# hku-mars/Voxel-SLAM

Measured on AMD Instinct MI355X. Metric: BA iterations/sec (10-frame window, 100k pts/scan), higher is better.
Workload: dtype f64; 1 GPU; cfg2: W=10, 100000 pts/scan, 50000 voxels per GPU, nnz=500000; global_voxels=50000, parallelism=voxel-shard x1, ranks_seen=1, collectives_per_lm_step=0, allreduce_doubles=0, lm_steps_accepted=2028, lm_steps_rejected=0

## Files before the change

### voxel-slam_amd/csrc/vxba_solve4.hpp

```cpp
#pragma once

typedef double s4v2 __attribute__((ext_vector_type(2)));

constexpr int S4_WAVES = 4;
constexpr int S4_THREADS = 64 * S4_WAVES;
constexpr int S4_ROW = 6;
constexpr int S4_BLK = 64 * S4_ROW + 6;
constexpr int S4_GSLOT = 64 * S4_ROW;

template <int W>
struct S4 {
  static constexpr int N = 6 * W, M = N - 6, B = W - 1;
  static constexpr int TC = 0;
  static constexpr int G = TC + (B > 0 ? B : 1) * S4_BLK;
  static constexpr int BV = G + (B > 0 ? B : 1) * S4_GSLOT;
  static constexpr int ZV = BV + 64;
  static constexpr int XS = ZV + 64;
  static constexpr int DOUBLES = XS + 64;
};

__device__ __forceinline__ double s4_rcp(double d) {
  const double r = __builtin_amdgcn_rcp(d);
  const double e = fma(-d, r, 1.0);
  const double t = fma(e, e, e);
  const double q = fma(r, t, r);
  return fabs(d) > 1e-300 ? q : 0.0;
}

__device__ __forceinline__ void s4_ldl6(double (&D)[21], double (&inv)[6]) {
#pragma unroll
  for (int p = 0; p < 6; p++) {
    inv[p] = s4_rcp(D[p * (p + 1) / 2 + p]);
    double col[6];
#pragma unroll
    for (int q = p + 1; q < 6; q++) col[q] = D[q * (q + 1) / 2 + p];
#pragma unroll
    for (int q = p + 1; q < 6; q++) {
      const double l = col[q] * inv[p];
#pragma unroll
      for (int r = p + 1; r <= q; r++) D[q * (q + 1) / 2 + r] = fma(-l, col[r], D[q * (q + 1) / 2 + r]);
      D[q * (q + 1) / 2 + p] = l;
    }
  }
}

__device__ __forceinline__ void s4_load_row(const double* p, double (&a)[6]) {
  const s4v2* v = reinterpret_cast<const s4v2*>(p);
  const s4v2 t0 = v[0], t1 = v[1], t2 = v[2];
  a[0] = t0[0]; a[1] = t0[1]; a[2] = t1[0]; a[3] = t1[1]; a[4] = t2[0]; a[5] = t2[1];
}
__device__ __forceinline__ void s4_store_row(double* p, const double (&a)[6]) {
  s4v2* v = reinterpret_cast<s4v2*>(p);
  v[0] = (s4v2){a[0], a[1]};
  v[1] = (s4v2){a[2], a[3]};
  v[2] = (s4v2){a[4], a[5]};
}

template <int W>
__device__ __forceinline__ void s4_apply(const double* lds, int t, int b, int lane, double (&T)[6]) {
  using C = S4<W>;
  double g[6];
  s4_load_row(lds + C::G + t * S4_GSLOT + lane * S4_ROW, g);
  const double* lr = lds + C::TC + t * S4_BLK + (6 * b) * S4_ROW;
#pragma unroll
  for (int c = 0; c < 6; c++) {
    double l[6];
    s4_load_row(lr + c * S4_ROW, l);
#pragma unroll
    for (int p = 0; p < 6; p++) T[c] = fma(-g[p], l[p], T[c]);
  }
}

constexpr int li_rec_len(int W) { return 1 + 12 * W + 6 * W + 36 * W * W; }
constexpr int li_out_len(int W) { return 6 * W + 12 * W + 1; }
template <int W, bool DBG>
__device__ __forceinline__ int lm_solve_body4(LMState* st, int c, double* lds, const double* __restrict__ li_rec = nullptr, double* __restrict__ li_out = nullptr,
                                               unsigned li_seq = 0) {
  using C = S4<W>;
  LMCtl& ctl = st->ctl[c];
  const int loop_done = ctl.done;
  constexpr int n = C::N, M = C::M, B = C::B;
  const int tid = threadIdx.x, lane = tid & 63;
  const int wave = __builtin_amdgcn_readfirstlane(tid >> 6);
  dbg_stamp(DBG && wave == 0, 4000, 0);
  dbg_stamp(DBG && wave == 0, 4000, 1);
  const double u = li_rec ? li_rec[0] : ctl.u;
  const double* __restrict__ li_x = li_rec ? li_rec + 1 : nullptr;
  const double* __restrict__ li_e = li_rec ? li_rec + 1 + 12 * W : nullptr;
  const double* __restrict__ li_E = li_rec ? li_rec + 1 + 18 * W : nullptr;
  const bool row_ok = lane < M;
  const int gi_row = row_ok ? 6 + lane : 0;

  constexpr int NQ = (B + S4_WAVES - 1) / S4_WAVES;
  double a0[NQ > 0 ? NQ : 1][6];
#pragma unroll
  for (int q = 0; q < NQ; q++) {
    const int b = wave + S4_WAVES * q;
    const int bb = b < B ? b : 0;
#pragma unroll
    for (int cc = 0; cc < 6; cc++) {
      const int col = 6 + 6 * bb + cc;
      const double h = st->Hwork[(size_t)col * n + gi_row];
      const double add = (li_E && gi_row >= 6 + 6 * bb) ? li_E[(size_t)col * n + gi_row] : 0.0;
      a0[q][cc] = row_ok ? (((col == gi_row) ? h + u * h : h) + add) : 0.0;
    }
  }
  double hii = 0.0, gi = 0.0, rhs0 = 0.0;
  double xcur[12];
  if (wave == 0) {
    hii = st->Hwork[(size_t)gi_row * n + gi_row];
    gi = st->Jwork[gi_row];
    const int fl = lane < W ? lane : 0;
#pragma unroll
    for (int k = 0; k < 12; k++) xcur[k] = li_x ? li_x[12 * fl + k] : ctl.x[12 * fl + k];
  }
  if (wave == 1 % S4_WAVES) rhs0 = row_ok ? (li_e ? li_e[gi_row] : 0.0) - st->Jwork[gi_row] : 0.0;
  if (loop_done) return 1;
  if (wave < B) s4_store_row(lds + C::TC + wave * S4_BLK + lane * S4_ROW, a0[0]);
  dbg_stamp(DBG && wave == 0, 4000, 2);

  int ap0 = -1, ap1 = -1, ap2 = -1;
  for (int s = 0; s < B; s++) {
    const int owner = s & (S4_WAVES - 1);
    double Ld[21], inv[6], g[6];
    if (wave == owner) {
      const int sq = s >> 2;
      const int ap = sq == 0 ? ap0 : (sq == 1 ? ap1 : ap2);
      double* trow = lds + C::TC + s * S4_BLK + lane * S4_ROW;
      double a[6];
      dbg_stamp(DBG, 4010 + s, 0);
      s4_load_row(trow, a);
      for (int t = ap + 1; t < s; t++) s4_apply<W>(lds, t, s, lane, a);
      if (DBG) { asm volatile("" :: "v"(a[0]), "v"(a[5])); dbg_stamp(true, 4010 + s, 1); }
      s4_store_row(trow, a);
      __builtin_amdgcn_wave_barrier();
      {
        const double* dr = lds + C::TC + s * S4_BLK + (6 * s) * S4_ROW;
        const s4v2 r0 = *reinterpret_cast<const s4v2*>(dr);
        const s4v2 r1 = *reinterpret_cast<const s4v2*>(dr + 6);
        const s4v2 r2a = *reinterpret_cast<const s4v2*>(dr + 12), r2b = *reinterpret_cast<const s4v2*>(dr + 14);
        const s4v2 r3a = *reinterpret_cast<const s4v2*>(dr + 18), r3b = *reinterpret_cast<const s4v2*>(dr + 20);
        const s4v2 r4a = *reinterpret_cast<const s4v2*>(dr + 24), r4b = *reinterpret_cast<const s4v2*>(dr + 26), r4c = *reinterpret_cast<const s4v2*>(dr + 28);
        const s4v2 r5a = *reinterpret_cast<const s4v2*>(dr + 30), r5b = *reinterpret_cast<const s4v2*>(dr + 32), r5c = *reinterpret_cast<const s4v2*>(dr + 34);
        Ld[0] = r0[0];
        Ld[1] = r1[0]; Ld[2] = r1[1];
        Ld[3] = r2a[0]; Ld[4] = r2a[1]; Ld[5] = r2b[0];
        Ld[6] = r3a[0]; Ld[7] = r3a[1]; Ld[8] = r3b[0]; Ld[9] = r3b[1];
        Ld[10] = r4a[0]; Ld[11] = r4a[1]; Ld[12] = r4b[0]; Ld[13] = r4b[1]; Ld[14] = r4c[0];
        Ld[15] = r5a[0]; Ld[16] = r5a[1]; Ld[17] = r5b[0]; Ld[18] = r5b[1]; Ld[19] = r5c[0]; Ld[20] = r5c[1];
      }
      if (DBG) { asm volatile("" :: "v"(Ld[0]), "v"(Ld[20])); dbg_stamp(true, 4010 + s, 2); }
      s4_ldl6(Ld, inv);
      if (DBG) { asm volatile("" :: "v"(inv[5])); dbg_stamp(true, 4010 + s, 3); }
      double l[6];
#pragma unroll
      for (int p = 0; p < 6; p++) {
        double acc = a[p];
#pragma unroll
        for (int q = 0; q < p; q++) acc = fma(-g[q], Ld[p * (p + 1) / 2 + q], acc);
        g[p] = acc;
        l[p] = acc * inv[p];
      }
      s4_store_row(trow, l);
      s4_store_row(lds + C::G + s * S4_GSLOT + lane * S4_ROW, g);
      if (sq == 0) ap0 = s; else if (sq == 1) ap1 = s; else ap2 = s;
      dbg_stamp(DBG, 4010 + s, 4);
    }
    if (s == 0) {
#pragma unroll
      for (int q = 1; q < NQ; q++) {
        const int b = wave + S4_WAVES * q;
        if (b < B) s4_store_row(lds + C::TC + b * S4_BLK + lane * S4_ROW, a0[q]);
      }
      if (wave == 1 % S4_WAVES) lds[C::BV + lane] = rhs0;
    }
    if (s < 9) dbg_stamp(DBG, 4000 + wave, 6 + 2 * s);
    __syncthreads();
    if (s < 9) dbg_stamp(DBG, 4000 + wave, 7 + 2 * s);
    if (wave == owner) {
      double bb[6];
      s4_load_row(lds + C::BV + 6 * s, bb);
      double br = lds[C::BV + lane];
      double z[6];
#pragma unroll
      for (int p = 0; p < 6; p++) {
        double acc = bb[p];
#pragma unroll
        for (int q = 0; q < p; q++) acc = fma(-bb[q], Ld[p * (p + 1) / 2 + q], acc);
        bb[p] = acc;
        z[p] = acc * inv[p];
      }
#pragma unroll
      for (int p = 0; p < 6; p++) br = fma(-g[p], z[p], br);
      const int d = lane - 6 * s;
      double zsel = z[0];
#pragma unroll
      for (int p = 1; p < 6; p++) zsel = (d == p) ? z[p] : zsel;
      if (d >= 0 && d < 6) lds[C::ZV + lane] = zsel;
      else lds[C::BV + lane] = br;
    }
    const bool next_owner = (s + 1 < B) && wave == ((s + 1) & (S4_WAVES - 1));
    if (!next_owner) {
      int budget = 2;
#pragma unroll
      for (int q = 0; q < (B + S4_WAVES - 1) / S4_WAVES; q++) {
        const int b = wave + S4_WAVES * q;
        int ap = q == 0 ? ap0 : (q == 1 ? ap1 : ap2);
        const bool must = b == s + 2;
        if (b > s && b < B && ap < s && (must || budget > 0)) {
          double* trow = lds + C::TC + b * S4_BLK + lane * S4_ROW;
          double T[6];
          s4_load_row(trow, T);
          while (ap < s && (must || budget > 0)) {
            s4_apply<W>(lds, ap + 1, b, lane, T);
            ap++;
            budget--;
          }
          s4_store_row(trow, T);
          if (q == 0) ap0 = ap; else if (q == 1) ap1 = ap; else ap2 = ap;
        }
      }
    }
  }
  __syncthreads();
  dbg_stamp(DBG && wave == 0, 4000, 3);
  if (wave != 0) return 0;

  double x = row_ok ? lds[C::ZV + lane] : 0.0;
  if constexpr (B > 0) {
    const int jb = (row_ok ? lane : 0) / 6, jc = (row_ok ? lane : 0) % 6;
    const double* lcol = lds + C::TC + jb * S4_BLK + jc;
    double Lr[6], Ln[6];
#pragma unroll
    for (int k = 0; k < 6; k++) Lr[k] = lcol[(M - 1 - k) * S4_ROW];
    for (int rb = B - 1; rb >= 0; rb--) {
      if (rb > 0) {
#pragma unroll
        for (int k = 0; k < 6; k++) Ln[k] = lcol[(6 * rb - 1 - k) * S4_ROW];
      }
#pragma unroll
      for (int k = 0; k < 6; k++) {
        const int r = 6 * rb + 5 - k;
        const double xr = readlane_f64(x, r);
        x = (lane < r) ? fma(-Lr[k], xr, x) : x;
      }
#pragma unroll
      for (int k = 0; k < 6; k++) Lr[k] = Ln[k];
    }
  }
  dbg_stamp(DBG, 4000, 4);
  if (row_ok) st->dxi[6 + lane] = x;
  if (lane < 6) st->dxi[lane] = 0.0;
  double* xs = lds + C::XS;
  if (lane < 6) xs[lane] = 0.0;
  if (row_ok) xs[6 + lane] = x;
  __builtin_amdgcn_wave_barrier();
  if (lane < W) {
    double dl[6];
#pragma unroll
    for (int k = 0; k < 6; k++) dl[k] = xs[6 * lane + k];
    double xn[9];
    lm_right_multiply_exp(xcur, dl, xn);
#pragma unroll
    for (int k = 0; k < 9; k++) __hip_atomic_store(&ctl.xt[12 * lane + k], xn[k], __ATOMIC_RELAXED, __HIP_MEMORY_SCOPE_AGENT);
#pragma unroll
    for (int k = 0; k < 3; k++) __hip_atomic_store(&ctl.xt[12 * lane + 9 + k], xcur[9 + k] + dl[3 + k], __ATOMIC_RELAXED, __HIP_MEMORY_SCOPE_AGENT);
    if (li_out) {
#pragma unroll
      for (int k = 0; k < 9; k++) li_out[6 * W + 12 * lane + k] = xn[k];
#pragma unroll
      for (int k = 0; k < 3; k++) li_out[6 * W + 12 * lane + 9 + k] = xcur[9 + k] + dl[3 + k];
    }
  }
  if (li_out) {
    if (row_ok) li_out[6 + lane] = x;
    if (lane < 6) li_out[lane] = 0.0;
    asm volatile("s_waitcnt vmcnt(0)" ::: "memory");
    __builtin_amdgcn_wave_barrier();
    if (lane == 0) li_out[18 * W] = (double)li_seq;
  }
  double part = row_ok ? x * (u * hii * x - gi) : 0.0;
#pragma unroll
  for (int off = 32; off > 0; off >>= 1) part += __shfl_down(part, off);
  if (lane == 0) ctl.q1 = 0.5 * part;
  if (DBG) { asm volatile("s_waitcnt vmcnt(0)" ::: "memory"); dbg_stamp(true, 4000, 5); }
  return 0;
}
```

Before: 21430 iterations/s.

## Keep block-Cholesky critical chain on wave 0 with register-carried next panel

```diff
diff --git a/voxel-slam_amd/csrc/vxba_solve4.hpp b/voxel-slam_amd/csrc/vxba_solve4.hpp
--- a/voxel-slam_amd/csrc/vxba_solve4.hpp
+++ b/voxel-slam_amd/csrc/vxba_solve4.hpp
@@ -69,6 +69,104 @@
 #pragma unroll
     for (int p = 0; p < 6; p++) T[c] = fma(-g[p], l[p], T[c]);
   }
+}
+
+template <int W>
+__device__ __forceinline__ void s4_apply_g(const double* lds, const double (&g)[6], int t, int b, double (&T)[6]) {
+  using C = S4<W>;
+  const double* lr = lds + C::TC + t * S4_BLK + (6 * b) * S4_ROW;
+#pragma unroll
+  for (int c = 0; c < 6; c++) {
+    double l[6];
+    s4_load_row(lr + c * S4_ROW, l);
+#pragma unroll
+    for (int p = 0; p < 6; p++) T[c] = fma(-g[p], l[p], T[c]);
+  }
+}
+
+template <int W>
+__device__ __forceinline__ void s4_rhs_step(double* lds, int s, int lane, const double (&Ld)[21], const double (&inv)[6], const double (&g)[6]) {
+  using C = S4<W>;
+  double bb[6];
+  s4_load_row(lds + C::BV + 6 * s, bb);
+  double br = lds[C::BV + lane];
+  double z[6];
+#pragma unroll
+  for (int p = 0; p < 6; p++) {
+    double acc = bb[p];
+#pragma unroll
+    for (int q = 0; q < p; q++) acc = fma(-bb[q], Ld[p * (p + 1) / 2 + q], acc);
+    bb[p] = acc;
+    z[p] = acc * inv[p];
+  }
+#pragma unroll
+  for (int p = 0; p < 6; p++) br = fma(-g[p], z[p], br);
+  const int d = lane - 6 * s;
+  double zsel = z[0];
+#pragma unroll
+  for (int p = 1; p < 6; p++) zsel = (d == p) ? z[p] : zsel;
+  const bool own = d >= 0 && d < 6;
+  lds[(own ? C::ZV : C::BV) + lane] = own ? zsel : br;
+}
+
+__device__ __forceinline__ void s4_stamp(bool on, int row, int slot) {
+  if (on) g_dbg[row * DBG_SLOTS + slot] = __builtin_readcyclecounter();
+}
+
+template <int W, bool DBG, bool FIRST, bool LAST>
+__device__ __forceinline__ void s4_chain_step(double* lds, int s, int lane, double (&a)[6], double (&nx)[6], double (&Ld)[21], double (&inv)[6], double (&g)[6]) {
+  using C = S4<W>;
+  double* trow = lds + C::TC + s * S4_BLK + lane * S4_ROW;
+  s4_stamp(DBG, 4010 + s, 0);
+  s4_store_row(trow, a);
+  __builtin_amdgcn_wave_barrier();
+  double Dn[21], invn[6], gn[6], l[6];
+  {
+    const double* dr = lds + C::TC + s * S4_BLK + (6 * s) * S4_ROW;
+    const s4v2 r0 = *reinterpret_cast<const s4v2*>(dr);
+    const s4v2 r1 = *reinterpret_cast<const s4v2*>(dr + 6);
+    const s4v2 r2a = *reinterpret_cast<const s4v2*>(dr + 12), r2b = *reinterpret_cast<const s4v2*>(dr + 14);
+    const s4v2 r3a = *reinterpret_cast<const s4v2*>(dr + 18), r3b = *reinterpret_cast<const s4v2*>(dr + 20);
+    const s4v2 r4a = *reinterpret_cast<const s4v2*>(dr + 24), r4b = *reinterpret_cast<const s4v2*>(dr + 26), r4c = *reinterpret_cast<const s4v2*>(dr + 28);
+    const s4v2 r5a = *reinterpret_cast<const s4v2*>(dr + 30), r5b = *reinterpret_cast<const s4v2*>(dr + 32), r5c = *reinterpret_cast<const s4v2*>(dr + 34);
+    Dn[0] = r0[0];
+    Dn[1] = r1[0]; Dn[2] = r1[1];
+    Dn[3] = r2a[0]; Dn[4] = r2a[1]; Dn[5] = r2b[0];
+    Dn[6] = r3a[0]; Dn[7] = r3a[1]; Dn[8] = r3b[0]; Dn[9] = r3b[1];
+    Dn[10] = r4a[0]; Dn[11] = r4a[1]; Dn[12] = r4b[0]; Dn[13] = r4b[1]; Dn[14] = r4c[0];
+    Dn[15] = r5a[0]; Dn[16] = r5a[1]; Dn[17] = r5b[0]; Dn[18] = r5b[1]; Dn[19] = r5c[0]; Dn[20] = r5c[1];
+  }
+  if constexpr (!FIRST) {
+    s4_rhs_step<W>(lds, s - 1, lane, Ld, inv, g);
+    if constexpr (!LAST) {
+      s4_load_row(lds + C::TC + (s + 1) * S4_BLK + lane * S4_ROW, nx);
+      s4_apply_g<W>(lds, g, s - 1, s + 1, nx);
+    }
+  }
+  if (DBG) { if (!FIRST && !LAST) asm volatile("" :: "v"(nx[0]), "v"(nx[5])); s4_stamp(true, 4010 + s, 1); }
+  if (DBG) { asm volatile("" :: "v"(Dn[0]), "v"(Dn[20])); s4_stamp(true, 4010 + s, 2); }
+  s4_ldl6(Dn, invn);
+  if (DBG) { asm volatile("" :: "v"(invn[5])); s4_stamp(true, 4010 + s, 3); }
+#pragma unroll
+  for (int p = 0; p < 6; p++) {
+    double acc = a[p];
+#pragma unroll
+    for (int q = 0; q < p; q++) acc = fma(-gn[q], Dn[p * (p + 1) / 2 + q], acc);
+    gn[p] = acc;
+    l[p] = acc * invn[p];
+  }
+  s4_store_row(trow, l);
+  __builtin_amdgcn_wave_barrier();
+  if constexpr (!LAST) {
+    s4_apply_g<W>(lds, gn, s, s + 1, nx);
+#pragma unroll
+    for (int k = 0; k < 6; k++) a[k] = nx[k];
+  }
+#pragma unroll
+  for (int k = 0; k < 21; k++) Ld[k] = Dn[k];
+#pragma unroll
+  for (int k = 0; k < 6; k++) { inv[k] = invn[k]; g[k] = gn[k]; }
+  s4_stamp(DBG, 4010 + s, 4);
 }
 
 constexpr int li_rec_len(int W) { return 1 + 12 * W + 6 * W + 36 * W * W; }
@@ -91,12 +189,13 @@
   const bool row_ok = lane < M;
   const int gi_row = row_ok ? 6 + lane : 0;
 
-  constexpr int NQ = (B + S4_WAVES - 1) / S4_WAVES;
-  double a0[NQ > 0 ? NQ : 1][6];
+  constexpr int NQH = (B - 2 + (S4_WAVES - 1) - 1) / (S4_WAVES - 1) > 0 ? (B - 2 + (S4_WAVES - 1) - 1) / (S4_WAVES - 1) : 0;
+  constexpr int NQ = NQH > 2 ? NQH : 2;
+  double a0[NQ][6];
 #pragma unroll
   for (int q = 0; q < NQ; q++) {
-    const int b = wave + S4_WAVES * q;
-    const int bb = b < B ? b : 0;
+    const int b = wave == 0 ? q : 1 + wave + (S4_WAVES - 1) * q;
+    const int bb = (b < B && (wave != 0 || q < 2)) ? b : 0;
 #pragma unroll
     for (int cc = 0; cc < 6; cc++) {
       const int col = 6 + 6 * bb + cc;
@@ -113,118 +212,63 @@
     const int fl = lane < W ? lane : 0;
 #pragma unroll
     for (int k = 0; k < 12; k++) xcur[k] = li_x ? li_x[12 * fl + k] : ctl.x[12 * fl + k];
-  }
-  if (wave == 1 % S4_WAVES) rhs0 = row_ok ? (li_e ? li_e[gi_row] : 0.0) - st->Jwork[gi_row] : 0.0;
+    rhs0 = row_ok ? (li_e ? li_e[gi_row] : 0.0) - gi : 0.0;
+  }
   if (loop_done) return 1;
-  if (wave < B) s4_store_row(lds + C::TC + wave * S4_BLK + lane * S4_ROW, a0[0]);
   dbg_stamp(DBG && wave == 0, 4000, 2);
 
-  int ap0 = -1, ap1 = -1, ap2 = -1;
-  for (int s = 0; s < B; s++) {
-    const int owner = s & (S4_WAVES - 1);
+  if (wave == 0) {
     double Ld[21], inv[6], g[6];
-    if (wave == owner) {
-      const int sq = s >> 2;
-      const int ap = sq == 0 ? ap0 : (sq == 1 ? ap1 : ap2);
-      double* trow = lds + C::TC + s * S4_BLK + lane * S4_ROW;
-      double a[6];
-      dbg_stamp(DBG, 4010 + s, 0);
-      s4_load_row(trow, a);
-      for (int t = ap + 1; t < s; t++) s4_apply<W>(lds, t, s, lane, a);
-      if (DBG) { asm volatile("" :: "v"(a[0]), "v"(a[5])); dbg_stamp(true, 4010 + s, 1); }
-      s4_store_row(trow, a);
-      __builtin_amdgcn_wave_barrier();
-      {
-        const double* dr = lds + C::TC + s * S4_BLK + (6 * s) * S4_ROW;
-        const s4v2 r0 = *reinterpret_cast<const s4v2*>(dr);
-        const s4v2 r1 = *reinterpret_cast<const s4v2*>(dr + 6);
-        const s4v2 r2a = *reinterpret_cast<const s4v2*>(dr + 12), r2b = *reinterpret_cast<const s4v2*>(dr + 14);
-        const s4v2 r3a = *reinterpret_cast<const s4v2*>(dr + 18), r3b = *reinterpret_cast<const s4v2*>(dr + 20);
-        const s4v2 r4a = *reinterpret_cast<const s4v2*>(dr + 24), r4b = *reinterpret_cast<const s4v2*>(dr + 26), r4c = *reinterpret_cast<const s4v2*>(dr + 28);
-        const s4v2 r5a = *reinterpret_cast<const s4v2*>(dr + 30), r5b = *reinterpret_cast<const s4v2*>(dr + 32), r5c = *reinterpret_cast<const s4v2*>(dr + 34);
-        Ld[0] = r0[0];
-        Ld[1] = r1[0]; Ld[2] = r1[1];
-        Ld[3] = r2a[0]; Ld[4] = r2a[1]; Ld[5] = r2b[0];
-        Ld[6] = r3a[0]; Ld[7] = r3a[1]; Ld[8] = r3b[0]; Ld[9] = r3b[1];
-        Ld[10] = r4a[0]; Ld[11] = r4a[1]; Ld[12] = r4b[0]; Ld[13] = r4b[1]; Ld[14] = r4c[0];
-        Ld[15] = r5a[0]; Ld[16] = r5a[1]; Ld[17] = r5b[0]; Ld[18] = r5b[1]; Ld[19] = r5c[0]; Ld[20] = r5c[1];
+    if constexpr (B > 0) lds[C::BV + lane] = rhs0;
+    for (int s = 0; s < B; s++) {
+      if (s == 0) s4_chain_step<W, DBG, true, B == 1>(lds, s, lane, a0[0], a0[1], Ld, inv, g);
+      else if (s == B - 1) s4_chain_step<W, DBG, false, true>(lds, s, lane, a0[0], a0[1], Ld, inv, g);
+      else s4_chain_step<W, DBG, false, false>(lds, s, lane, a0[0], a0[1], Ld, inv, g);
+      if (s + 2 < B) {
+        s4_store_row(lds + C::G + s * S4_GSLOT + lane * S4_ROW, g);
+        if (s < 9) dbg_stamp(DBG, 4000 + wave, 6 + 2 * s);
+        __syncthreads();
+        if (s < 9) dbg_stamp(DBG, 4000 + wave, 7 + 2 * s);
       }
-      if (DBG) { asm volatile("" :: "v"(Ld[0]), "v"(Ld[20])); dbg_stamp(true, 4010 + s, 2); }
-      s4_ldl6(Ld, inv);
-      if (DBG) { asm volatile("" :: "v"(inv[5])); dbg_stamp(true, 4010 + s, 3); }
-      double l[6];
-#pragma unroll
-      for (int p = 0; p < 6; p++) {
-        double acc = a[p];
-#pragma unroll
-        for (int q = 0; q < p; q++) acc = fma(-g[q], Ld[p * (p + 1) / 2 + q], acc);
-        g[p] = acc;
-        l[p] = acc * inv[p];
-      }
-      s4_store_row(trow, l);
-      s4_store_row(lds + C::G + s * S4_GSLOT + lane * S4_ROW, g);
-      if (sq == 0) ap0 = s; else if (sq == 1) ap1 = s; else ap2 = s;
-      dbg_stamp(DBG, 4010 + s, 4);
-    }
-    if (s == 0) {
-#pragma unroll
-      for (int q = 1; q < NQ; q++) {
-        const int b = wave + S4_WAVES * q;
-        if (b < B) s4_store_row(lds + C::TC + b * S4_BLK + lane * S4_ROW, a0[q]);
-      }
-      if (wave == 1 % S4_WAVES) lds[C::BV + lane] = rhs0;
-    }
-    if (s < 9) dbg_stamp(DBG, 4000 + wave, 6 + 2 * s);
-    __syncthreads();
-    if (s < 9) dbg_stamp(DBG, 4000 + wave, 7 + 2 * s);
-    if (wave == owner) {
-      double bb[6];
-      s4_load_row(lds + C::BV + 6 * s, bb);
-      double br = lds[C::BV + lane];
-      double z[6];
-#pragma unroll
-      for (int p = 0; p < 6; p++) {
-        double acc = bb[p];
-#pragma unroll
-        for (int q = 0; q < p; q++) acc = fma(-bb[q], Ld[p * (p + 1) / 2 + q], acc);
-        bb[p] = acc;
-        z[p] = acc * inv[p];
-      }
-#pragma unroll
-      for (int p = 0; p < 6; p++) br = fma(-g[p], z[p], br);
-      const int d = lane - 6 * s;
-      double zsel = z[0];
-#pragma unroll
-      for (int p = 1; p < 6; p++) zsel = (d == p) ? z[p] : zsel;
-      if (d >= 0 && d < 6) lds[C::ZV + lane] = zsel;
-      else lds[C::BV + lane] = br;
-    }
-    const bool next_owner = (s + 1 < B) && wave == ((s + 1) & (S4_WAVES - 1));
-    if (!next_owner) {
-      int budget = 2;
-#pragma unroll
-      for (int q = 0; q < (B + S4_WAVES - 1) / S4_WAVES; q++) {
-        const int b = wave + S4_WAVES * q;
-        int ap = q == 0 ? ap0 : (q == 1 ? ap1 : ap2);
-        const bool must = b == s + 2;
-        if (b > s && b < B && ap < s && (must || budget > 0)) {
-          double* trow = lds + C::TC + b * S4_BLK + lane * S4_ROW;
-          double T[6];
-          s4_load_row(trow, T);
-          while (ap < s && (must || budget > 0)) {
-            s4_apply<W>(lds, ap + 1, b, lane, T);
-            ap++;
-            budget--;
+    }
+    if constexpr (B > 0) s4_rhs_step<W>(lds, B - 1, lane, Ld, inv, g);
+  } else {
+    int ap0 = -1, ap1 = -1, ap2 = -1;
+    for (int s = 0; s + 2 < B; s++) {
+      if (s == 0) {
+#pragma unroll
+        for (int q = 0; q < NQH; q++) {
+          const int b = 1 + wave + (S4_WAVES - 1) * q;
+          if (b < B) s4_store_row(lds + C::TC + b * S4_BLK + lane * S4_ROW, a0[q]);
+        }
+      } else {
+        int budget = 2;
+#pragma unroll
+        for (int q = 0; q < NQH; q++) {
+          const int b = 1 + wave + (S4_WAVES - 1) * q;
+          int ap = q == 0 ? ap0 : (q == 1 ? ap1 : ap2);
+          const bool must = b == s + 2;
+          if (b >= s + 2 && b < B && ap < s - 1 && (must || budget > 0)) {
+            double* trow = lds + C::TC + b * S4_BLK + lane * S4_ROW;
+            double T[6];
+            s4_load_row(trow, T);
+            while (ap < s - 1 && (must || budget > 0)) {
+              s4_apply<W>(lds, ap + 1, b, lane, T);
+              ap++;
+              budget--;
+            }
+            s4_store_row(trow, T);
+            if (q == 0) ap0 = ap; else if (q == 1) ap1 = ap; else ap2 = ap;
           }
-          s4_store_row(trow, T);
-          if (q == 0) ap0 = ap; else if (q == 1) ap1 = ap; else ap2 = ap;
         }
       }
-    }
-  }
-  __syncthreads();
-  dbg_stamp(DBG && wave == 0, 4000, 3);
-  if (wave != 0) return 0;
+      if (s < 9) dbg_stamp(DBG, 4000 + wave, 6 + 2 * s);
+      __syncthreads();
+      if (s < 9) dbg_stamp(DBG, 4000 + wave, 7 + 2 * s);
+    }
+    return 0;
+  }
+  dbg_stamp(DBG, 4000, 3);
 
   double x = row_ok ? lds[C::ZV + lane] : 0.0;
   if constexpr (B > 0) {
```

After: 20280 iterations/s. -5.4%, worse.
